# JiGuang283/Ray_Tracing-Rendering

Hardware: AMD Instinct MI355X
Metric: Msamples/sec, Cornell Box 800x800 spp=400 MIS (higher is better)
Workload: dtype f64

## Files before the change

### ray_tracing-rendering_amd/csrc/rt_device.h

```cpp
#pragma once

#include <hip/hip_runtime.h>
#include <stdint.h>

#include "rtr_hip.h"
#include "rtr_seed.h"

#ifndef RTR_BLOCK
#define RTR_BLOCK 256
#endif

#define RT_DEV __device__ __forceinline__
#define RT_HD __host__ __device__ __forceinline__

typedef double Real;

#define RT_STATS_WORDS 80
#define RT_PROF_BASE 8
#define RT_PROF_REGIONS 36
enum { RG_OTHER = 0, RG_SETUP = 1, RG_RECTS = 2, RG_SPHERES = 3, RG_GENERIC = 4, RG_TREE = 5, RG_LEAVES = 6, RG_FINISH = 7,
       RG_SH_SETUP = 8, RG_SH_RECTS = 9, RG_SH_SPHERES = 10, RG_SH_GENERIC = 11, RG_SH_TREE = 12, RG_SH_LEAVES = 13,
       RG_MEDIA = 14, RG_MATPREP = 15, RG_SHADE_A = 16, RG_SHADE_B = 17, RG_MISS = 18, RG_REGEN = 19, RG_SHADE_RR = 20,
       RG_PARK = 21, RG_BARRIER = 22, RG_EXCHANGE = 23, RG_PAIR_SETUP = 24, RG_PAIR_RUNS = 25, RG_PAIR_SPHERES = 26,
       RG_POLL = 27, RG_BEGIN = 28, RG_SETTLE = 29, RG_COUNT = 30, RG_REJECT = 31,
       RG_EMIT_MIS = 32,
       RG_CAMDIV = 33,
       RG_LANE_DIV = 34,
       RG_LANE_SQRT = 35,
       RG_N = 36 };
#ifdef RTR_REGION_PROFILE
__shared__ unsigned long long rt_prof_lds[4 * 2 * RT_PROF_REGIONS + 4 * 2];
RT_DEV void rt_region(int id) {
    const unsigned long long m = __ballot(1);
    if ((int)__lane_id() == __builtin_ctzll(m)) {
        const int w = threadIdx.x >> 6;
        unsigned long long* acc = rt_prof_lds + w * 2 * RT_PROF_REGIONS;
        unsigned long long* st = rt_prof_lds + 4 * 2 * RT_PROF_REGIONS + w * 2;
        const unsigned long long now = __builtin_readcyclecounter();
        acc[st[1]] += now - st[0];
        acc[RT_PROF_REGIONS + id] += 1;
        st[0] = now, st[1] = (unsigned long long)id;
    }
}
RT_DEV int rt_region_current() { return (int)rt_prof_lds[4 * 2 * RT_PROF_REGIONS + (threadIdx.x >> 6) * 2 + 1]; }
#define RT_REGION(id) rt_region(id)
#define RT_REGION_CURRENT() rt_region_current()
#else
#define RT_REGION(id) do { } while (0)
#define RT_REGION_CURRENT() 0
#endif

#define RT_INF (__builtin_huge_val())
// ... 1404 lines not shown
                 ".Lpx%=:\n\t"
                 "s_mov_b64 exec, %[save]"
                 : [u] "=&v"(u), [save] "=&s"(save), [tmaxA] "+v"(tmaxA), [hitA] "+v"(hitA), [tmaxB] "+v"(tmaxB), [hitB] "+v"(hitB)
                 : [tA] "v"(tA), [uA] "v"(uA), [wA] "v"(wA), [tB] "v"(tB), [oaB] "v"(oaB), [daB] "v"(daB), [obB] "v"(obB),
                   [dbB] "v"(dbB), [a0] "s"(a0), [a1] "s"(a1), [b0] "s"(b0), [b1] "s"(b1), [ref] "s"(ref), [tmin] "s"(tmin)
                 : "vcc");
}
struct PairRay {
    V3 o, d;
    RayDiv q;
};
template <int TYPE>
RT_DEV void pair_rects(const RT_CONST_AS double* p, int cnt, int ref, const PairRay& A, Real& tmaxA, int& hitA, const PairRay& B,
                       Real& tmaxB, int& hitB) {
    int k = 0;
    for (; k + 1 < cnt; k += 2, p += 10) {
        const Real f0 = p[0], f1 = p[1], f2 = p[2], f3 = p[3], f4 = p[4];
        const Real g0 = p[5], g1 = p[6], g2 = p[7], g3 = p[8], g4 = p[9];
        pair_rect<TYPE>(f0, f1, f2, f3, f4, ref + k, A.o, A.d, A.q, tmaxA, hitA, B.o, B.d, B.q, tmaxB, hitB);
        pair_rect<TYPE>(g0, g1, g2, g3, g4, ref + k + 1, A.o, A.d, A.q, tmaxA, hitA, B.o, B.d, B.q, tmaxB, hitB);
    }
    if (k < cnt) pair_rect<TYPE>(p[0], p[1], p[2], p[3], p[4], ref + k, A.o, A.d, A.q, tmaxA, hitA, B.o, B.d, B.q, tmaxB, hitB);
}
RT_DEV void pair_runs(const DScene& sc, const FInst& I, const PairRay& A, Real time, Real& tmaxA, int& hitA, const PairRay& B,
                      Real& tmaxB, int& hitB) {
    const RT_CONST_AS double* p = as_const(sc.fscan) + I.scan_first;
    int ref = I.ref_first;
#pragma nounroll
    for (uint64_t runs = I.runs; runs != 0; runs >>= RT_RUN_BITS) {
        const int type = RTR_NODE_SPHERE + (int)((runs >> RT_RUN_COUNT_BITS) & 7), cnt = (int)(runs & RT_RUN_COUNT_MAX);
        RT_REGION(type >= RTR_NODE_XY_RECT ? RG_PAIR_RUNS : RG_PAIR_SPHERES);
        if (type == RTR_NODE_XY_RECT) {
            pair_rects<RTR_NODE_XY_RECT>(p, cnt, ref, A, tmaxA, hitA, B, tmaxB, hitB);
            p += 5 * cnt;
        } else if (type == RTR_NODE_XZ_RECT) {
            pair_rects<RTR_NODE_XZ_RECT>(p, cnt, ref, A, tmaxA, hitA, B, tmaxB, hitB);
            p += 5 * cnt;
        } else if (type == RTR_NODE_YZ_RECT) {
            pair_rects<RTR_NODE_YZ_RECT>(p, cnt, ref, A, tmaxA, hitA, B, tmaxB, hitB);
            p += 5 * cnt;
        } else if (type == RTR_NODE_SPHERE + RT_RUN_BOX) {
            for (int b = 0, r = ref; b < cnt; ++b, p += 6, r += 6) {
                const Real x0 = p[0], x1 = p[1], y0 = p[2], y1 = p[3], z0 = p[4], z1 = p[5];
                pair_rect<RTR_NODE_XY_RECT>(x0, x1, y0, y1, z1, r, A.o, A.d, A.q, tmaxA, hitA, B.o, B.d, B.q, tmaxB, hitB);
                pair_rect<RTR_NODE_XY_RECT>(x0, x1, y0, y1, z0, r + 1, A.o, A.d, A.q, tmaxA, hitA, B.o, B.d, B.q, tmaxB, hitB);
                pair_rect<RTR_NODE_XZ_RECT>(x0, x1, z0, z1, y1, r + 2, A.o, A.d, A.q, tmaxA, hitA, B.o, B.d, B.q, tmaxB, hitB);
                pair_rect<RTR_NODE_XZ_RECT>(x0, x1, z0, z1, y0, r + 3, A.o, A.d, A.q, tmaxA, hitA, B.o, B.d, B.q, tmaxB, hitB);
                pair_rect<RTR_NODE_YZ_RECT>(y0, y1, z0, z1, x1, r + 4, A.o, A.d, A.q, tmaxA, hitA, B.o, B.d, B.q, tmaxB, hitB);
                pair_rect<RTR_NODE_YZ_RECT>(y0, y1, z0, z1, x0, r + 5, A.o, A.d, A.q, tmaxA, hitA, B.o, B.d, B.q, tmaxB, hitB);
            }
            ref += 5 * cnt;
        } else {
            for (int k = 0; k < cnt; ++k, p += 4) {
                const V3 c = mk(p[0], p[1], p[2]);
                const Real r = p[3];
                Real t;
                if (sphere_hit_t<true>(c, r, A.o, A.d, A.q, 0.001, tmaxA, t)) tmaxA = t, hitA = ref + k;
                if (sphere_hit_t<true>(c, r, B.o, B.d, B.q, 0.001, tmaxB, t)) tmaxB = t, hitB = ref + k;
            }
        }
        ref += cnt;
    }
}
struct PairFrame {
    V3 ao, bo;
    Real adx, adz, bdx, bdz;
};
RT_HD void pair_rot(Real s, Real c, Real x, Real z, Real& rx, Real& rz) {
    rx = c * x - s * z;
    rz = s * x + c * z;
}
RT_HD PairFrame pair_frame(int shape, const double* f0, const double* f1, V3 ao, V3 ad, V3 bo, V3 bd) {
    PairFrame F;
    switch (shape) {
    case RT_SHAPE_T:
// ... 11 lines not shown
        const Real ax = ao.x - f0[0], bx = bo.x - f0[0];
        const Real az = ao.z - f0[2], bz = bo.z - f0[2];
        F.ao.y = ao.y - f0[1], F.bo.y = bo.y - f0[1];
        pair_rot(f1[0], f1[1], ax, az, F.ao.x, F.ao.z), pair_rot(f1[0], f1[1], bx, bz, F.bo.x, F.bo.z);
        pair_rot(f1[0], f1[1], ad.x, ad.z, F.adx, F.adz), pair_rot(f1[0], f1[1], bd.x, bd.z, F.bdx, F.bdz);
        break;
    }
    case RT_SHAPE_RT: {
        Real ax, az, bx, bz;
        pair_rot(f0[0], f0[1], ao.x, ao.z, ax, az), pair_rot(f0[0], f0[1], bo.x, bo.z, bx, bz);
        pair_rot(f0[0], f0[1], ad.x, ad.z, F.adx, F.adz), pair_rot(f0[0], f0[1], bd.x, bd.z, F.bdx, F.bdz);
        F.ao.x = ax - f1[0], F.bo.x = bx - f1[0];
        F.ao.y = ao.y - f1[1], F.bo.y = bo.y - f1[1];
        F.ao.z = az - f1[2], F.bo.z = bz - f1[2];
        break;
    }
    default:
        F.ao = ao, F.bo = bo;
        F.adx = ad.x, F.adz = ad.z, F.bdx = bd.x, F.bdz = bd.z;
        break;
    }
    return F;
}
__device__ __forceinline__ void trace_pair(const DScene& sc, V3 ao, V3 ad, Real atime, Real& a_tmax, int& a_ref, int& a_inst,
                                           V3 bo, V3 bd, Real& b_tmax, int& b_ref, const Stack st) {
    a_ref = -1, a_inst = -1, b_ref = -1;
#ifndef RTR_NO_SHARED_DIV
    const bool ok_a = raydiv_origin_ok(ao), ok_b = raydiv_origin_ok(bo);
#else
    const bool ok_a = false, ok_b = false;
#endif
    const Real way = rcp_refined(ad.y), wby = rcp_refined(bd.y);
    const bool wa_y = rcp_safe(ad.y), wb_y = rcp_safe(bd.y);
    for (int ii = 0; ii < sc.n_finst; ++ii) {
        RT_REGION(RG_PAIR_SETUP);
        const FInst I = ld_const(sc.finst, ii);
        PairRay A, B;
        if (I.shape != RT_SHAPE_OTHER) {
            const PairFrame F = pair_frame(I.shape, I.xf_f[0], I.xf_f[1], ao, ad, bo, bd);
            A.o = F.ao, B.o = F.bo;
            A.d = mk(F.adx, ad.y, F.adz), B.d = mk(F.bdx, bd.y, F.bdz);
        } else {
            A.o = ao, A.d = ad, B.o = bo, B.d = bd;
            wrapper_enter(I.xf_type[0], I.xf_f[0], A.o, A.d);
            wrapper_enter(I.xf_type[0], I.xf_f[0], B.o, B.d);
            if (I.n_xf > 1) {
                wrapper_enter(I.xf_type[1], I.xf_f[1], A.o, A.d);
                wrapper_enter(I.xf_type[1], I.xf_f[1], B.o, B.d);
// ... 13 lines not shown
        if (I.flags & RT_INST_SPHERES) {
            A.q.a = len2(A.d), B.q.a = len2(B.d);
            A.q.ra = rcp_refined(A.q.a), B.q.ra = rcp_refined(B.q.a);
            sa = sa & rcp_safe(A.q.a), sb = sb & rcp_safe(B.q.a);
        }
        if (ok_a && ok_b && __all(sa & sb)) {
            A.q.fast = B.q.fast = true;
            pair_runs(sc, I, A, atime, a_tmax, a_ref, B, b_tmax, b_ref);
        } else {
            A.q.fast = ok_a && __all(sa), B.q.fast = ok_b && __all(sb);
            int order = -1;
            if (A.q.fast)
                scan_instance<false, false, false, true>(sc, I, A.o, A.d, A.q, atime, 0.001, a_tmax, a_ref, order, st, 0);
            else
                scan_instance<false, false, false, false>(sc, I, A.o, A.d, A.q, atime, 0.001, a_tmax, a_ref, order, st, 0);
            if (B.q.fast)
                scan_instance<true, false, true, true>(sc, I, B.o, B.d, B.q, 0.0, 0.001, b_tmax, b_ref, order, st, 0);
            else
                scan_instance<true, false, true, false>(sc, I, B.o, B.d, B.q, 0.0, 0.001, b_tmax, b_ref, order, st, 0);
        }
        RT_REGION(RG_PAIR_SETUP);
        if (a_ref >= I.ref_first) a_inst = ii;
    }
}

template <bool UV>
__device__ __forceinline__ void fast_finish_long(const DScene& sc, V3 o, V3 d, Real time, Real t, int ref, int inst, Hit& rec) {
    const FInst I = ld_const(sc.finst, inst);
    const FRef R = ld_const(sc.fref, ref);
    V3 lo = o, ld = d;
    for (int k = 0; k < I.n_xf; ++k) {
        const FXf x = ld_const(sc.fxf, I.xf_first + k);
        wrapper_enter(x.type, x.f, lo, ld);
    }
    const rtr_node n = ld_const(sc.fprim, ref);
    const int type = n.type;
    if (type >= RTR_NODE_XY_RECT) {
        Real oa, da, ob, db;
        if (type == RTR_NODE_XY_RECT) {
            oa = lo.x, da = ld.x, ob = lo.y, db = ld.y;
        } else if (type == RTR_NODE_XZ_RECT) {
            oa = lo.x, da = ld.x, ob = lo.z, db = ld.z;
        } else {
            oa = lo.y, da = ld.y, ob = lo.z, db = ld.z;
        }
        rect_fill(n, type, lo, ld, t, oa + t * da, ob + t * db, UV, rec);
// ... 1166 lines not shown
```

### ray_tracing-rendering_amd/csrc/rt_kernels.h

```cpp
#pragma once

#include "rt_render.h"

#ifndef RTR_MEGA_WAVES
#define RTR_MEGA_WAVES 4
#endif
#ifndef RTR_PROGRAM_WAVES
#define RTR_PROGRAM_WAVES 3
#endif

constexpr int mega_waves(int integ, int trav, int ms) {
    if (ms == RT_MS_LEAN) return RTR_MEGA_WAVES;
    if (rt_is_program(trav)) return RTR_PROGRAM_WAVES;
    if (trav == RT_TRAV_MEDIA || trav == RT_TRAV_EXACT) return 2;
    if (ms == RT_MS_QUADLIT) return 3;
    if (integ == RTR_INTEGRATOR_RR || integ == RTR_INTEGRATOR_PATH) return 3;
    return 2;
}

#define RT_PARK_WORDS 19
struct Park {
    double* base;
    RT_DEV V3 get3(int k) const { return mk(base[k * RTR_BLOCK], base[(k + 1) * RTR_BLOCK], base[(k + 2) * RTR_BLOCK]); }
    RT_DEV void set3(int k, V3 v) const {
        base[k * RTR_BLOCK] = v.x, base[(k + 1) * RTR_BLOCK] = v.y, base[(k + 2) * RTR_BLOCK] = v.z;
    }
    RT_DEV double get(int k) const { return base[k * RTR_BLOCK]; }
    RT_DEV void set(int k, double v) const { base[k * RTR_BLOCK] = v; }
    RT_DEV void get2(int k, uint32_t& lo, uint32_t& hi) const {
        const unsigned long long w = (unsigned long long)__double_as_longlong(base[k * RTR_BLOCK]);
        lo = (uint32_t)w, hi = (uint32_t)(w >> 32);
    }
    RT_DEV void set2(int k, uint32_t lo, uint32_t hi) const {
        base[k * RTR_BLOCK] = __longlong_as_double((long long)((unsigned long long)lo | ((unsigned long long)hi << 32)));
    }
};
enum { PK_THR = 0, PK_L = 3, PK_ACC = 6, PK_PDF = 9, PK_NCAST = 10, PK_PIXEL = 11,
       PK_CONTRIB = 12, PK_SWI = 15, PK_STMAX = 18 };
struct ParkedReq {
    bool valid;
    Park pk;
// ... 300 lines not shown
            RTR_CLK(other);
            RT_REGION(RG_OTHER);
            const bool cast_a = !done;
            Real a_tmax = RT_INF, b_tmax = 0.0;
            int a_ref, a_inst, b_ref;
            V3 swi = mk(1.0, 1.0, 1.0);
            RT_REGION(RG_COUNT);
            {
                uint32_t n_closest, n_shadow;
                pk.get2(PK_NCAST, n_closest, n_shadow);
                pk.set2(PK_NCAST, n_closest + (cast_a ? 1u : 0u), n_shadow + (pending ? 1u : 0u));
            }
            RT_REGION(RG_OTHER);
            if (!cast_a) {
                ps.ro = mk(0.0, 0.0, 0.0), ps.rd = mk(1.0, 1.0, 1.0), ps.tm = 0.0;
                a_tmax = 0.0;
            }
            if (pending) {
                swi = pk.get3(PK_SWI);
                b_tmax = pk.get(PK_STMAX);
            } else {
                so = mk(0.0, 0.0, 0.0);
            }
            trace_pair(sc, ps.ro, ps.rd, ps.tm, a_tmax, a_ref, a_inst, so, swi, b_tmax, b_ref, st);
            RTR_CLK(closest);
            RT_REGION(RG_POLL);
            const uint32_t cancel_word = cancel_poll_issue(P, it++);
            RT_REGION(RG_SETTLE);
            const bool lit = pending && b_ref < 0;
            if (lit || settle) {
                V3 L = pk.get3(PK_L);
                if (lit) L = add(L, pk.get3(PK_CONTRIB));
                if (settle) {
                    pk.set3(PK_ACC, add(pk.get3(PK_ACC), L));
                    if (ACC == 2) {
                        const double y = luminance(L);
                        q += y * y;
                    }
                    L = mk(0.0, 0.0, 0.0);
                    settle = false;
                }
                pk.set3(PK_L, L);
            }
            pending = false;
            RTR_CLK(shadow);
            if (cast_a) {
                bool ended;
// ... 252 lines not shown
        bool now = false;
        if (need && k < RT_QUEUE_JOBS) {
            const int i = tile_x * 16 + (k & 15), j = tile_y * 16 + qb.quarter * 4 + (k >> 4);
            if (i >= P.x0 && i < P.x1 && j >= P.y0 && j < P.y1 && qb.s0 < qb.s1) {
                uint32_t lo, hi;
                queue_pack(i, j, qb.s1, lo, hi);
                pk.set2(PK_PIXEL, lo, hi);
                *my_cell = cell;
                s = qb.s0;
                got = now = true, need = false;
            } else {
                atomicAdd(&P.done[cell], 1);
            }
        }
        qw.samples += (unsigned long long)__builtin_popcountll(__ballot(now)) * (unsigned long long)(qb.s1 - qb.s0);
        const int taken = qw.next + (int)__builtin_popcountll(m);
        qw.next = taken < RT_QUEUE_JOBS ? taken : RT_QUEUE_JOBS;
        m = __ballot(need);
    }
    slot.set(qw);
    return got;
}

template <int INTEG, int TRAV, int MS>
__global__ void __launch_bounds__(RTR_BLOCK, mega_waves(INTEG, TRAV, MS))
    k_mega_queue(const DScene* __restrict__ scp, const RenderK P, const int stack_words, uint32_t* __restrict__ ,
                 const int ) {
    static_assert(mega_pairable(INTEG, TRAV), "no pair-cast variant of this kernel");
    extern __shared__ int lds_stack[];
    const DScene& sc = *scp;
    const Stack st{lds_stack + threadIdx.x};
    const Park pk{reinterpret_cast<double*>(lds_stack + stack_words * RTR_BLOCK) + threadIdx.x};
    int* const my_cell = lds_stack + threadIdx.x;
    const QueueSlot slot;
#ifdef RTR_REGION_PROFILE
    if (threadIdx.x < 4 * 2 * RT_PROF_REGIONS + 8) rt_prof_lds[threadIdx.x] = 0;
    if (threadIdx.x + 256 < 4 * 2 * RT_PROF_REGIONS + 8) rt_prof_lds[threadIdx.x + 256] = 0;
    __syncthreads();
    if ((threadIdx.x & 63) == 0) rt_prof_lds[4 * 2 * RT_PROF_REGIONS + (threadIdx.x >> 6) * 2] = __builtin_readcyclecounter();
#endif
    PathCounters cnt;
    cnt.closest = 0, cnt.shadow = 0;
    PathState ps;
    uint32_t rng = 1;
    int s = 0;
    slot.set(QueueWave{0, RT_QUEUE_JOBS, 0ull});
// ... 23 lines not shown
    bool pending = false;
    bool settle = false;
    V3 so = mk(0.0, 0.0, 0.0);
    PhaseClocks clk;
    while (!done || settle) {
        RTR_CLK(other);
        RT_REGION(RG_OTHER);
        const bool cast_a = !done;
        Real a_tmax = RT_INF;
        int a_ref, a_inst, b_ref;
        RT_REGION(RG_COUNT);
        {
            uint32_t n_closest, n_shadow;
            pk.get2(PK_NCAST, n_closest, n_shadow);
            pk.set2(PK_NCAST, n_closest + (cast_a ? 1u : 0u), n_shadow + (pending ? 1u : 0u));
        }
        RT_REGION(RG_OTHER);
        if (!cast_a) {
            ps.ro = mk(0.0, 0.0, 0.0), ps.rd = mk(1.0, 1.0, 1.0), ps.tm = 0.0;
            a_tmax = 0.0;
        }
        const V3 swi = pk.get3(PK_SWI);
        Real b_tmax = pk.get(PK_STMAX);
        trace_pair(sc, ps.ro, ps.rd, ps.tm, a_tmax, a_ref, a_inst, so, swi, b_tmax, b_ref, st);
        RTR_CLK(closest);
        RT_REGION(RG_POLL);
        const uint32_t cancel_word = cancel_poll_issue(P, it++);
        RT_REGION(RG_SETTLE);
        const bool lit = pending && b_ref < 0;
        if (lit || settle) {
            V3 L = pk.get3(PK_L);
            if (lit) L = add(L, pk.get3(PK_CONTRIB));
            if (settle) {
                pk.set3(PK_ACC, add(pk.get3(PK_ACC), L));
                L = mk(0.0, 0.0, 0.0);
                settle = false;
            }
            pk.set3(PK_L, L);
        }
        pending = false;
        {
            Real dead = 0.0;
            asm volatile("" : "+v"(dead));
            pk.set(PK_STMAX, dead);
        }
        RTR_CLK(shadow);
        bool begin = false;
// ... 542 lines not shown
```

### ray_tracing-rendering_amd/csrc/rt_test_kernels.h

```cpp
#pragma once

#include "rt_kernels.h"
#include "rtr_hip_test.h"
#include "rtr_testrec.h"

template <int TRAV>
__global__ void __launch_bounds__(RTR_BLOCK) k_test_hits(const DScene sc, rtr_hit_record* recs, long long n) {
    extern __shared__ int lds_stack[];
    const Stack st{lds_stack + threadIdx.x};
    const long long k = (long long)blockIdx.x * RTR_BLOCK + threadIdx.x;
    if (k >= n) return;
    rtr_hit_record r = recs[k];
    uint32_t rng = r.rng_in;
    Hit rec;
    rec.u = rec.v = __builtin_nan("");
    rec.mat = -1;
    rec.t = 0, rec.p = mk(0, 0, 0), rec.n = mk(0, 0, 0), rec.front = false;
    Real tmax = r.t_max;
    bool h;
    if (TRAV == RT_TRAV_FAST || TRAV == RT_TRAV_TOP) {
        int ref, inst;
        h = trace_fast<false, true, false, TRAV == RT_TRAV_TOP>(sc, sub_scene0(sc), ld3(r.o), ld3(r.d), r.time, r.t_min, tmax, ref, inst, st, 0);
        if (h) fast_finish<true>(sc, ld3(r.o), ld3(r.d), r.time, tmax, ref, inst, rec);
    } else if (rt_is_program(TRAV)) {
// ... 18 lines not shown
    extern __shared__ int lds_stack[];
    const Stack st{lds_stack + threadIdx.x};
    const long long k = (long long)blockIdx.x * RTR_BLOCK + threadIdx.x;
    if (k >= n) return;
    rtr_hit_record r = recs[k];
    uint32_t rng = r.rng_in;
    Hit rec;
    rec.u = rec.v = __builtin_nan("");
    rec.mat = -1;
    rec.t = 0, rec.p = mk(0, 0, 0), rec.n = mk(0, 0, 0), rec.front = false;
    const bool h = cast_closest<TRAV>(sc, ld3(r.o), ld3(r.d), r.time, rec, rng, st, r.t_min, r.t_max);
    r.rng_out = rng;
    r.hit = h;
    r.front_face = h ? (int)rec.front : 0;
    r.material = h ? rec.mat : -1;
    r.pad = 0;
    r.t = h ? rec.t : 0;
    r.p[0] = h ? rec.p.x : 0, r.p[1] = h ? rec.p.y : 0, r.p[2] = h ? rec.p.z : 0;
    r.n[0] = h ? rec.n.x : 0, r.n[1] = h ? rec.n.y : 0, r.n[2] = h ? rec.n.z : 0;
    r.u = h ? rec.u : 0, r.v = h ? rec.v : 0;
    recs[k] = r;
}

__global__ void __launch_bounds__(RTR_BLOCK) k_test_pair(const DScene sc, rtr_pair_record* recs, long long n) {
    extern __shared__ int lds_stack[];
    const Stack st{lds_stack + threadIdx.x};
    const long long k = (long long)blockIdx.x * RTR_BLOCK + threadIdx.x;
    if (k >= n) return;
    rtr_pair_record r = recs[k];
    Real a_t = r.a_tmax, b_t = r.b_tmax;
    int a_ref, a_inst, b_ref;
    trace_pair(sc, ld3(r.ao), ld3(r.ad), 0.0, a_t, a_ref, a_inst, ld3(r.bo), ld3(r.bd), b_t, b_ref, st);
    Real s_t = r.a_tmax, sb_t = r.b_tmax;
    int s_ref, s_inst, sb_ref, sb_inst;
    trace_fast<false, false, false, false, false>(sc, sub_scene0(sc), ld3(r.ao), ld3(r.ad), 0.0, 0.001, s_t, s_ref, s_inst, st, 0);
    trace_fast<true, false, true, false, false>(sc, sub_scene0(sc), ld3(r.bo), ld3(r.bd), 0.0, 0.001, sb_t, sb_ref, sb_inst, st, 0);
    r.a_t = a_t, r.s_a_t = s_t;
    r.a_ref = a_ref, r.a_inst = a_inst, r.b_hit = b_ref >= 0;
    r.s_a_ref = s_ref, r.s_a_inst = s_inst, r.s_b_hit = sb_ref >= 0;
    recs[k] = r;
}

RT_DEV bool same_bits(Real a, Real b) { return (a != a && b != b) || __double_as_longlong(a) == __double_as_longlong(b); }

template <int MS>
__global__ void __launch_bounds__(RTR_BLOCK) k_test_materials(const DScene sc, rtr_mat_record* recs, long long n) {
    const long long k = (long long)blockIdx.x * RTR_BLOCK + threadIdx.x;
    if (k >= n) return;
    rtr_mat_record r = recs[k];
    Hit rec;
    rec.p = ld3(r.p), rec.n = ld3(r.n);
    rec.u = r.u, rec.v = r.v, rec.t = 1.0;
    rec.front = r.front_face != 0;
    rec.mat = r.material;
    const V3 wo = ld3(r.wo), wi = ld3(r.wi_in);
    uint32_t rng = r.rng_in;
    BSDFSample bs;
    bs.wi = mk(0, 0, 0), bs.f = mk(0, 0, 0), bs.pdf = 0, bs.is_specular = false, bs.is_transmission = false;
    const MatCtx mc = mat_prepare<MS>(sc, rec);
    const UDiv pi = scene_pi(sc);
    const bool ok = mat_sample<MS>(mc, rec, wo, bs, rng, pi);
// ... 298 lines not shown
```

### ray_tracing-rendering_amd/csrc/rtr_capi.hip

```cpp
#include "rt_context.h"
#include "rt_render_kernels.h"
#include "rt_validate.h"

#include <cstdio>
#include <cstring>

using namespace rtr;

static thread_local std::string g_create_error;

namespace rtr {

int fail(rtr_context* c, int code, const std::string& msg) {
    if (c)
        c->err = msg;
    else
        g_create_error = msg;
    return code;
}

int ensure(rtr_context* c, DevBuf& b, size_t bytes) {
    if (bytes == 0) bytes = 16;
    if (b.cap >= bytes) return RTR_OK;
    if (b.p) {
// ... 73 lines not shown
            c->in_flight = false;
            HIPCHK(c, hipStreamSynchronize(c->stream));
        }
        return RTR_OK;
    }
    HIPCHK(c, hipEventSynchronize(c->ev1));
    float ms = 0;
    HIPCHK(c, hipEventElapsedTime(&ms, c->ev0, c->ev1));
    unsigned long long h[RT_STATS_WORDS] = {0};
    HIPCHK(c, hipMemcpy(h, c->b_stats.p, sizeof h, hipMemcpyDeviceToHost));
    if (getenv("RTR_REGION_PROFILE")) {
        static const char* names[RG_N] = {"other / loop", "closest: instance setup", "closest: rect runs", "closest: sphere runs",
                                          "closest: generic scan", "closest: tree inner nodes", "closest: tree leaves",
                                          "closest: hit record (fast_finish)", "shadow: instance setup", "shadow: rect runs",
                                          "shadow: sphere runs", "shadow: generic scan", "shadow: tree inner nodes",
                                          "shadow: tree leaves", "media steps", "mat_prepare", "shade_a (emission, light sample)",
                                          "shade_b (BSDF sample, roulette)", "miss", "end of sample + regeneration",
                                          "shade_rr / shade_path", "park path state", "sorted shading: barrier waits",
                                          "sorted shading: tickets + exchange / queue: job switch", "pair cast: instance setup",
                                          "pair cast: rect runs", "pair cast: sphere runs", "sample end: cancel poll",
                                          "sample end: begin_sample (camera ray)", "sample end: settle into the pixel sum",
                                          "cast counters", "random_in_unit_sphere rejection loop",
                                          "shade_a: emitter MIS weight (compute_light_pdf)", "camera_sample: image-size divisions",
                                          "shading: lane-varying 1 / x and n / d", "shading: lane-varying sqrt"};
        double total = 0;
        for (int k = 0; k < RG_N; ++k) total += (double)h[RT_PROF_BASE + k];
        std::fprintf(stderr, "[region profile] %.4g wave cycles in all, %llu samples\n", total, h[0]);
        for (int k = 0; k < RG_N; ++k)
            if (h[RT_PROF_BASE + RT_PROF_REGIONS + k])
                std::fprintf(stderr, "[region profile] %-48s %6.2f %%  %12llu visits  %8.1f cycles/visit\n", names[k],
                             100.0 * (double)h[RT_PROF_BASE + k] / total, h[RT_PROF_BASE + RT_PROF_REGIONS + k],
                             (double)h[RT_PROF_BASE + k] / (double)h[RT_PROF_BASE + RT_PROF_REGIONS + k]);
    }
#ifdef RTR_PHASE_CLOCKS
    std::fprintf(stderr, "[phase clocks] closest %.3e  shade %.3e  shadow %.3e  other %.3e (wave cycles)\n", (double)h[3],
                 (double)h[4], (double)h[5], (double)h[6]);
#endif
    c->stats.samples = h[0];
    c->stats.closest_segments = h[1];
    c->stats.shadow_segments = h[2];
    c->stats.device_ms = ms;
    if (h[7]) c->stats.cancelled = 1;
    c->stats_pending = false;
    c->in_flight = false;
    return RTR_OK;
}

// ... 616 lines not shown
```

### ray_tracing-rendering_amd/native.py

```python
import ctypes as C
import os
import weakref

import numpy as np

from . import _abi as A
from .scene import Scene

_HERE = os.path.dirname(os.path.abspath(__file__))
_LIB = None

_STATUS = {A.RTR_ERR_INVALID: "RTR_ERR_INVALID", A.RTR_ERR_UNSUPPORTED: "RTR_ERR_UNSUPPORTED",
           A.RTR_ERR_DEVICE: "RTR_ERR_DEVICE", A.RTR_ERR_NO_SCENE: "RTR_ERR_NO_SCENE",
           A.RTR_ERR_CANCELLED: "RTR_ERR_CANCELLED", A.RTR_ERR_NOMEM: "RTR_ERR_NOMEM"}

EXPORTS = ("rtr_abi_version", "rtr_device_count", "rtr_create", "rtr_destroy", "rtr_set_stream",
           "rtr_upload_scene", "rtr_render_device", "rtr_render_host", "rtr_render_tiles_host", "rtr_plan_chunks", "rtr_li_samples", "rtr_li_rays",
           "rtr_synchronize", "rtr_cancel", "rtr_get_stats", "rtr_last_error", "rtr_sample_seed", "rtr_validate_scene",
           "rtr_accum_create", "rtr_accum_render", "rtr_accum_resolve", "rtr_accum_tiles", "rtr_accum_destroy",
           "rtr_accum_create_ex", "rtr_accum_render_tiles", "rtr_accum_moments", "rtr_accum_errors", "rtr_accum_refine",
           "rtr_denoise_defaults", "rtr_accum_features", "rtr_accum_denoise", "rtr_denoise_host",
           "rtr_query_closest", "rtr_query_occluded", "rtr_query_closest_device", "rtr_query_occluded_device",
           "rtr_set_camera", "rtr_get_camera", "rtr_accum_reset", "rtr_temporal_defaults", "rtr_history_create",
           "rtr_history_clear", "rtr_history_destroy", "rtr_history_planes", "rtr_accum_denoise_temporal",
           "rtr_display_defaults", "rtr_display_srgb_thresholds", "rtr_display_histogram", "rtr_display_host",
           "rtr_display_device", "rtr_accum_resolve_device", "rtr_accum_features_device", "rtr_accum_denoise_device",
           "rtr_accum_denoise_temporal_device", "rtr_gather_defaults", "rtr_gather_occlusion", "rtr_gather_radiance",
           "rtr_gather_occlusion_device", "rtr_gather_radiance_device", "rtr_gather_ray",
           "rtr_probe_visibility", "rtr_probe_radiance", "rtr_probe_visibility_device", "rtr_probe_radiance_device",
           "rtr_probe_ray", "rtr_sh_basis", "rtr_sh_irradiance", "rtr_probe_lookup", "rtr_probe_lookup_device",
           "rtr_probe_lookup_one", "rtr_capture_defaults", "rtr_capture_cube", "rtr_capture_cube_device", "rtr_capture_ray",
           "rtr_cube_lookup", "rtr_cube_lookup_device", "rtr_cube_lookup_one", "rtr_latlong_direction",
           "rtr_cube_to_latlong", "rtr_write_rgbe", "rtr_cube_filter_defaults", "rtr_cube_filter", "rtr_cube_filter_device",
           "rtr_cube_filter_one", "rtr_cube_chain_plan", "rtr_cube_chain_lookup", "rtr_cube_chain_lookup_device",
           "rtr_cube_chain_lookup_one", "rtr_probe_depth_defaults", "rtr_probe_depth", "rtr_probe_depth_device",
           "rtr_probe_depth_ray", "rtr_octa_encode", "rtr_octa_decode", "rtr_probe_lookup_visible",
           "rtr_probe_lookup_visible_device", "rtr_probe_lookup_visible_one")
TEST_EXPORTS = ("rtr_test_hits", "rtr_test_materials", "rtr_test_lights", "rtr_test_li", "rtr_test_reference_order",
                "rtr_test_stream8", "rtr_test_sincos_exhaustive", "rtr_test_shared_division", "rtr_test_issue_rates", "rtr_test_last_kernel",
                "rtr_test_last_gather", "rtr_test_last_probe", "rtr_test_last_capture", "rtr_test_last_probe_depth",
                "rtr_test_temporal_planes", "rtr_test_scene_plan", "rtr_test_flat_hits", "rtr_test_pair_frames",
                "rtr_test_pair_frame_host", "rtr_test_pair_cast", "rtr_test_queue_blocks_host", "rtr_test_queue_pack_host",
                "rtr_test_scatter", "rtr_test_materials_ms", "rtr_test_scatter_ms", "rtr_test_lights_ms", "rtr_test_pow5",
                "rtr_test_pow5_host", "rtr_test_udiv", "rtr_test_scene_consts", "rtr_test_accum_load",
                "rtr_test_accum_plan", "rtr_test_accum_commit", "rtr_test_rcp_lane", "rtr_test_sqrt_lane",
                "rtr_test_lane_specials", "rtr_test_lane_host", "rtr_test_draw_forms", "rtr_test_draw_callers",
                "rtr_test_draw_host", "rtr_test_draw_host_range")
_TEST_LIB = None


class SceneInfoC(C.Structure):
    _fields_ = [("stack_words", C.c_int32), ("has_media", C.c_int32), ("needs_uv", C.c_int32),
                ("graph_depth", C.c_int32), ("fast_ok", C.c_int32), ("fast_instances", C.c_int32),
                ("fast_refs", C.c_int32), ("fast_stack_words", C.c_int32), ("compiled_subtrees", C.c_int32),
                ("program_steps", C.c_int32), ("inverted_boxes", C.c_int32), ("top_trees", C.c_int32)]


class KernelRecordC(C.Structure):
    _fields_ = [(name, C.c_int32) for name in ("pipeline", "integrator", "trav", "ms", "sorted", "shade_phases", "lean",
                                               "quadlit", "sort", "media", "machine", "accum", "pair", "queue")]


class GatherRecordC(C.Structure):
    _fields_ = [(name, C.c_int32) for name in ("integ", "trav", "broadcast", "lg")]

# ... 6 lines not shown
    _fields_ = [(name, C.c_int32) for name in ("integ", "trav", "lg")]


class ProbeDepthRecordC(C.Structure):
    _fields_ = [(name, C.c_int32) for name in ("trav", "lg")]


class ScenePlanC(C.Structure):
    _fields_ = [(name, C.c_int32) for name in (
        "fast_ok", "has_media", "flat_scene", "flat_guarded", "lean_materials", "quad_lights_only", "uv_order_dependent",
        "machine_ok", "guarded_program", "top_tree", "needs_uv", "n_material_types", "shared_div", "pair_cast", "n_steps",
        "n_visits", "n_refs", "fast_stack_words", "walk_stack_words", "n_tie_refs", "n_guard_refs", "pick_trav", "mega_trav",
        "mega_ms", "mega_sorted", "mega_pair", "n_finish")]


FINISH_DTYPE = np.dtype([("kind", "<i4"), ("material", "<i4"), ("levels", "<i4"), ("flip", "<i4"), ("op", "<f8", (2, 3)),
                         ("g", "<f8", (4,))])


PAIR_FRAME_DTYPE = np.dtype([("ao", "<f8", (3,)), ("ad", "<f8", (3,)), ("bo", "<f8", (3,)), ("bd", "<f8", (3,)),
                             ("fo", "<f8", (3,)), ("fd", "<f8", (3,)), ("same_frame", "<i4"), ("pad", "<i4")])
PAIR_DTYPE = np.dtype([("ao", "<f8", (3,)), ("ad", "<f8", (3,)), ("a_tmax", "<f8"), ("bo", "<f8", (3,)), ("bd", "<f8", (3,)),
                       ("b_tmax", "<f8"), ("a_t", "<f8"), ("s_a_t", "<f8"), ("a_ref", "<i4"), ("a_inst", "<i4"),
                       ("b_hit", "<i4"), ("s_a_ref", "<i4"), ("s_a_inst", "<i4"), ("s_b_hit", "<i4")])
QUEUE_BLOCK_DTYPE = np.dtype([(name, "<i4") for name in ("slot", "quarter", "chunk", "s0", "s1", "ref_s0", "ref_s1", "pad")])
MS_LEAN, MS_FULL, MS_QUADLIT = 0, 1, 2
FRAME_SHAPES = ("none", "T", "R", "TR", "RT", "other")


class RtrError(RuntimeError):
    def __init__(self, code, message):
        super().__init__("%s (%d): %s" % (_STATUS.get(code, "rtr_status"), code, message))
        self.code = code
        self.message = message


def library_path():
    return os.environ.get("RTR_HIP_LIBRARY") or os.path.join(_HERE, "librtr_hip.so")


def lib():
    global _LIB
    if _LIB is not None:
        return _LIB
    path = library_path()
    if not os.path.exists(path):
        raise RtrError(A.RTR_ERR_DEVICE, "HIP library %s is missing: run __graft_entry__.build(); there is no "
# ... 136 lines not shown
    for name in ("rtr_test_materials_ms", "rtr_test_scatter_ms", "rtr_test_lights_ms"):
        getattr(T, name).argtypes = [vp, vp, C.c_int64, C.c_int32]
    T.rtr_test_pow5.argtypes = [vp, vp, vp, C.c_int64]
    T.rtr_test_pow5_host.argtypes = [vp, vp, C.c_int64]
    T.rtr_test_li.argtypes = [vp, C.POINTER(A.RenderParamsC), vp, C.c_int64]
    T.rtr_test_reference_order.argtypes = [vp, C.c_int]
    T.rtr_test_stream8.argtypes = [vp, C.c_int64, C.c_int]
    T.rtr_test_sincos_exhaustive.argtypes = [vp, C.POINTER(C.c_uint64), C.POINTER(C.c_uint64)]
    T.rtr_test_issue_rates.argtypes = [vp, C.POINTER(C.c_double), C.c_int]
    T.rtr_test_shared_division.argtypes = [vp, C.POINTER(C.c_uint64), C.POINTER(C.c_uint64)]
    T.rtr_test_last_kernel.argtypes = [vp, C.POINTER(KernelRecordC), C.c_size_t]
    T.rtr_test_last_gather.argtypes = [vp, C.POINTER(GatherRecordC), C.c_size_t]
    T.rtr_test_last_probe.argtypes = [vp, C.POINTER(ProbeRecordC), C.c_size_t]
    T.rtr_test_last_capture.argtypes = [vp, C.POINTER(CaptureRecordC), C.c_size_t]
    T.rtr_test_last_probe_depth.argtypes = [vp, C.POINTER(ProbeDepthRecordC), C.c_size_t]
    T.rtr_test_temporal_planes.argtypes = [vp] + [C.c_int32] * 6 + [C.POINTER(A.CameraC), C.POINTER(A.CameraC), C.c_int,
                                                                    C.POINTER(A.TemporalParamsC)] + [vp] * 8
    T.rtr_test_scene_plan.argtypes = [C.POINTER(A.SceneDescC), C.c_int32, C.c_int32, C.POINTER(ScenePlanC), vp, C.c_int64,
                                      vp, C.c_int64]
    T.rtr_test_flat_hits.argtypes = [vp, vp, C.c_int64, C.c_int, C.POINTER(C.c_int32)]
    T.rtr_test_pair_frames.argtypes = [C.POINTER(A.SceneDescC), vp, C.c_int64, C.POINTER(C.c_int32)]
    T.rtr_test_pair_frame_host.argtypes = [C.c_int32, vp, vp, C.c_int64]
    T.rtr_test_pair_cast.argtypes = [vp, vp, C.c_int64]
    T.rtr_test_queue_blocks_host.argtypes = [C.c_int32] * 6 + [vp, C.c_int64]
    T.rtr_test_queue_pack_host.argtypes = [C.c_int32] * 3 + [C.POINTER(C.c_uint32), C.POINTER(C.c_uint32), vp]
    T.rtr_test_udiv.argtypes = [vp, vp, C.c_int64, vp, C.c_int32, C.POINTER(C.c_uint64), C.POINTER(C.c_uint64)]
    T.rtr_test_scene_consts.argtypes = [vp, vp, vp, C.c_int64, C.POINTER(C.c_int32)]
    for name in ("rtr_test_rcp_lane", "rtr_test_sqrt_lane"):
        getattr(T, name).argtypes = [vp] + [C.POINTER(C.c_uint64)] * 3 + [vp]
    T.rtr_test_lane_specials.argtypes = [vp, C.c_int64]
    T.rtr_test_lane_host.argtypes = [C.c_int32, C.c_int32, vp, vp, vp, C.c_int64]
    T.rtr_test_draw_forms.argtypes = [vp] + [C.POINTER(C.c_uint64)] * 3
    T.rtr_test_draw_callers.argtypes = [vp, C.c_uint64, C.c_int64] + [C.POINTER(C.c_uint64)] * 3
    T.rtr_test_draw_host.argtypes = [vp, vp, C.c_int64]
    T.rtr_test_draw_host_range.argtypes = [C.c_uint64, C.c_uint64, C.c_uint64, C.c_int32, C.POINTER(C.c_uint64), C.POINTER(C.c_uint64)]
    T.rtr_test_accum_load.argtypes = [vp, vp, vp, vp, vp, C.c_int64]
    T.rtr_test_accum_plan.argtypes = [vp, C.c_int64] + [C.c_int32] * 4 + [C.c_double, vp, vp, vp, vp, C.POINTER(C.c_int32)]
    T.rtr_test_accum_commit.argtypes = [vp, C.c_int64, vp, C.c_int32] + [vp] * 7
    _TEST_LIB = T
    return T


def validate_scene(scene):
    L = lib()
    d = scene.desc()
    info = SceneInfoC()
# ... 1026 lines not shown
        sum_ = np.array(sum, dtype=np.float64, order="C")
        cnt = np.array(count, dtype=np.int32, order="C")
        if any(a.shape != (n,) for a in ints) or cnt.shape != (n,) or partial.shape != (n, 3, 256) or sum_.shape != (n, 3, 256):
            raise ValueError("n tiles: int arrays (n,), partial and sum (n, 3, 256) expected")
        if (q is None) != (q_part is None):
            raise ValueError("q and q_part go together")
        qq = qp = None
        if q is not None:
            qp = np.ascontiguousarray(q_part, dtype=np.float64)
            qq = np.array(q, dtype=np.float64, order="C")
            if qp.shape != (n, 256) or qq.shape != (n, 256):
                raise ValueError("q_part and q of shape (n, 256) expected")
        self._chk(test_lib().rtr_test_accum_commit(
            self._h, n, ints[0].ctypes.data, int(n_active), ints[1].ctypes.data, ints[2].ctypes.data, partial.ctypes.data,
            None if qp is None else qp.ctypes.data, sum_.ctypes.data, None if qq is None else qq.ctypes.data, cnt.ctypes.data))
        return sum_, qq, cnt

    def flat_hits(self, recs, with_uv=True):
        out = np.ascontiguousarray(recs.copy())
        used = C.c_int32(0)
        self._chk(test_lib().rtr_test_flat_hits(self._h, out.ctypes.data, len(out), 1 if with_uv else 0, C.byref(used)))
        return out, bool(used.value)

    def pair_cast(self, ao, ad, bo, bd, a_tmax=np.inf, b_tmax=np.inf):
        recs = np.zeros(len(ao), dtype=PAIR_DTYPE)
        recs["ao"], recs["ad"], recs["bo"], recs["bd"] = ao, ad, bo, bd
        recs["a_tmax"], recs["b_tmax"] = a_tmax, b_tmax
        self._chk(test_lib().rtr_test_pair_cast(self._h, recs.ctypes.data, len(recs)))
        return recs

    def test_records(self, kind, recs, params=None, ms=None):
        out = np.ascontiguousarray(recs.copy())
        if kind == "pow5":
            x = np.ascontiguousarray(recs, dtype=np.float64)
            out = np.zeros_like(x)
            self._chk(test_lib().rtr_test_pow5(self._h, x.ctypes.data, out.ctypes.data, x.size))
            return out
        if ms is not None:
            fn = getattr(test_lib(), "rtr_test_%s_ms" % kind)
            self._chk(fn(self._h, out.ctypes.data, len(out), int(ms)))
            return out
        fn = getattr(test_lib(), "rtr_test_" + kind)
        if kind == "li":
            self._chk(fn(self._h, C.byref(params), out.ctypes.data, len(out)))
        else:
            self._chk(fn(self._h, out.ctypes.data, len(out)))
        return out


class Accumulator:

# ... 200 lines not shown
```

Baseline: 6073.

## Add lean pair-cast path that bails to single casts when fast-division checks fail

Result: faster. 6215, median of 6 (+2.3%).

```diff
diff --git a/ray_tracing-rendering_amd/csrc/rt_device.h b/ray_tracing-rendering_amd/csrc/rt_device.h
--- a/ray_tracing-rendering_amd/csrc/rt_device.h
+++ b/ray_tracing-rendering_amd/csrc/rt_device.h
@@ -15,9 +15,9 @@
 
 typedef double Real;
 
-#define RT_STATS_WORDS 80
+#define RT_STATS_WORDS 82
 #define RT_PROF_BASE 8
-#define RT_PROF_REGIONS 36
+#define RT_PROF_REGIONS 37
 enum { RG_OTHER = 0, RG_SETUP = 1, RG_RECTS = 2, RG_SPHERES = 3, RG_GENERIC = 4, RG_TREE = 5, RG_LEAVES = 6, RG_FINISH = 7,
        RG_SH_SETUP = 8, RG_SH_RECTS = 9, RG_SH_SPHERES = 10, RG_SH_GENERIC = 11, RG_SH_TREE = 12, RG_SH_LEAVES = 13,
        RG_MEDIA = 14, RG_MATPREP = 15, RG_SHADE_A = 16, RG_SHADE_B = 17, RG_MISS = 18, RG_REGEN = 19, RG_SHADE_RR = 20,
@@ -27,7 +27,8 @@
        RG_CAMDIV = 33,
        RG_LANE_DIV = 34,
        RG_LANE_SQRT = 35,
-       RG_N = 36 };
+       RG_PAIR_RECAST = 36,
+       RG_N = 37 };
 #ifdef RTR_REGION_PROFILE
 __shared__ unsigned long long rt_prof_lds[4 * 2 * RT_PROF_REGIONS + 4 * 2];
 RT_DEV void rt_region(int id) {
@@ -1478,6 +1479,7 @@
     }
     if (k < cnt) pair_rect<TYPE>(p[0], p[1], p[2], p[3], p[4], ref + k, A.o, A.d, A.q, tmaxA, hitA, B.o, B.d, B.q, tmaxB, hitB);
 }
+template <bool SPHERES = true>
 RT_DEV void pair_runs(const DScene& sc, const FInst& I, const PairRay& A, Real time, Real& tmaxA, int& hitA, const PairRay& B,
                       Real& tmaxB, int& hitB) {
     const RT_CONST_AS double* p = as_const(sc.fscan) + I.scan_first;
@@ -1506,7 +1508,7 @@
                 pair_rect<RTR_NODE_YZ_RECT>(y0, y1, z0, z1, x0, r + 5, A.o, A.d, A.q, tmaxA, hitA, B.o, B.d, B.q, tmaxB, hitB);
             }
             ref += 5 * cnt;
-        } else {
+        } else if (SPHERES) {
             for (int k = 0; k < cnt; ++k, p += 4) {
                 const V3 c = mk(p[0], p[1], p[2]);
                 const Real r = p[3];
@@ -1564,8 +1566,8 @@
     }
     return F;
 }
-__device__ __forceinline__ void trace_pair(const DScene& sc, V3 ao, V3 ad, Real atime, Real& a_tmax, int& a_ref, int& a_inst,
-                                           V3 bo, V3 bd, Real& b_tmax, int& b_ref, const Stack st) {
+__device__ __forceinline__ bool trace_pair_frames(const DScene& sc, V3 ao, V3 ad, Real atime, Real& a_tmax, int& a_ref, int& a_inst,
+                                                  V3 bo, V3 bd, Real& b_tmax, int& b_ref, const Stack st) {
     a_ref = -1, a_inst = -1, b_ref = -1;
 #ifndef RTR_NO_SHARED_DIV
     const bool ok_a = raydiv_origin_ok(ao), ok_b = raydiv_origin_ok(bo);
@@ -1625,6 +1627,100 @@
         RT_REGION(RG_PAIR_SETUP);
         if (a_ref >= I.ref_first) a_inst = ii;
     }
+    return true;
+}
+typedef unsigned long long PairMask;
+RT_DEV PairMask pair_within(Real x, Real lo, Real hi) {
+    PairMask a, b;
+    asm volatile("v_cmp_ge_f64_e64 %0, |%2|, %3\n\tv_cmp_le_f64_e64 %1, |%2|, %4" : "=&s"(a), "=&s"(b) : "v"(x), "s"(lo), "s"(hi));
+    return a & b;
+}
+RT_DEV PairMask pair_safe(Real d) { return pair_within(d, 0x1p-100, 0x1p100); }
+RT_DEV PairMask pair_below(Real x, Real hi) {
+    PairMask a;
+    asm volatile("v_cmp_le_f64_e64 %0, |%1|, %2" : "=s"(a) : "v"(x), "s"(hi));
+    return a;
+}
+RT_DEV PairMask pair_origin_in(V3 o) { return pair_below(o.x, 0x1p80) & pair_below(o.y, 0x1p80) & pair_below(o.z, 0x1p80); }
+RT_DEV bool pair_vote(PairMask m) { return m == __builtin_amdgcn_read_exec(); }
+RT_DEV bool pair_scan(const DScene& sc, const FInst& I, V3 ao, Real adx, Real ady, Real adz, Real way, V3 bo, Real bdx, Real bdy,
+                      Real bdz, Real wby, PairMask sy, Real atime, Real& a_tmax, int& a_ref, Real& b_tmax, int& b_ref) {
+    PairRay A, B;
+    A.o = ao, B.o = bo;
+    A.d = mk(adx, ady, adz), B.d = mk(bdx, bdy, bdz);
+    A.q.guard = B.q.guard = false;
+    A.q.fast = B.q.fast = true;
+    A.q.rx = rcp_refined(adx), A.q.rz = rcp_refined(adz);
+    B.q.rx = rcp_refined(bdx), B.q.rz = rcp_refined(bdz);
+    A.q.ry = way, B.q.ry = wby;
+    A.q.a = A.q.ra = B.q.a = B.q.ra = 0;
+    const PairMask s = pair_safe(adx) & pair_safe(adz) & pair_safe(bdx) & pair_safe(bdz) & sy;
+    if (I.flags & RT_INST_SPHERES) {
+        Real ayy, byy;
+        asm volatile("v_mul_f64 %0, %2, %2\n\tv_mul_f64 %1, %3, %3" : "=&v"(ayy), "=&v"(byy) : "v"(ady), "v"(bdy));
+        A.q.a = adx * adx + ayy + adz * adz, B.q.a = bdx * bdx + byy + bdz * bdz;
+        A.q.ra = rcp_refined(A.q.a), B.q.ra = rcp_refined(B.q.a);
+        if (!pair_vote(s & pair_safe(A.q.a) & pair_safe(B.q.a))) return false;
+        pair_runs<true>(sc, I, A, atime, a_tmax, a_ref, B, b_tmax, b_ref);
+    } else {
+        if (!pair_vote(s)) return false;
+        pair_runs<false>(sc, I, A, atime, a_tmax, a_ref, B, b_tmax, b_ref);
+    }
+    return true;
+}
+__device__ __forceinline__ bool trace_pair_recast(const DScene& sc, V3 ao, V3 ad, Real atime, Real& a_tmax, int& a_ref, int& a_inst,
+                                                  V3 bo, V3 bd, Real& b_tmax, int& b_ref) {
+    a_ref = -1, a_inst = -1, b_ref = -1;
+#ifdef RTR_NO_SHARED_DIV
+    return false;
+#endif
+    if (!pair_vote(pair_origin_in(ao) & pair_origin_in(bo))) return false;
+    const Real way = rcp_refined(ad.y), wby = rcp_refined(bd.y);
+    const PairMask sy = pair_safe(ad.y) & pair_safe(bd.y);
+    for (int ii = 0; ii < sc.n_finst; ++ii) {
+        RT_REGION(RG_PAIR_SETUP);
+        const FInst I = ld_const(sc.finst, ii);
+        PairFrame F;
+        if (I.shape != RT_SHAPE_OTHER) {
+            F = pair_frame(I.shape, I.xf_f[0], I.xf_f[1], ao, ad, bo, bd);
+        } else {
+            V3 fad = ad, fbd = bd;
+            F.ao = ao, F.bo = bo;
+            wrapper_enter(I.xf_type[0], I.xf_f[0], F.ao, fad);
+            wrapper_enter(I.xf_type[0], I.xf_f[0], F.bo, fbd);
+            if (I.n_xf > 1) {
+                wrapper_enter(I.xf_type[1], I.xf_f[1], F.ao, fad);
+                wrapper_enter(I.xf_type[1], I.xf_f[1], F.bo, fbd);
+            }
+            for (int k = RT_INST_XF_INLINE; k < I.n_xf; ++k) {
+                const FXf x = ld_const(sc.fxf, I.xf_first + k);
+                wrapper_enter(x.type, x.f, F.ao, fad);
+                wrapper_enter(x.type, x.f, F.bo, fbd);
+            }
+            F.adx = fad.x, F.adz = fad.z, F.bdx = fbd.x, F.bdz = fbd.z;
+        }
+        if (!pair_scan(sc, I, F.ao, F.adx, ad.y, F.adz, way, F.bo, F.bdx, bd.y, F.bdz, wby, sy, atime, a_tmax, a_ref, b_tmax, b_ref))
+            return false;
+        RT_REGION(RG_PAIR_SETUP);
+        if (a_ref >= I.ref_first) a_inst = ii;
+    }
+    return true;
+}
+template <bool RECAST = true>
+__device__ __forceinline__ bool trace_pair(const DScene& sc, V3 ao, V3 ad, Real atime, Real& a_tmax, int& a_ref, int& a_inst,
+                                           V3 bo, V3 bd, Real& b_tmax, int& b_ref, const Stack st) {
+#ifndef RTR_PAIR_FRAME_FALLBACK
+    if (RECAST) return trace_pair_recast(sc, ao, ad, atime, a_tmax, a_ref, a_inst, bo, bd, b_tmax, b_ref);
+#endif
+    return trace_pair_frames(sc, ao, ad, atime, a_tmax, a_ref, a_inst, bo, bd, b_tmax, b_ref, st);
+}
+RT_DEV void pair_recast(const DScene& sc, V3 ao, V3 ad, Real atime, Real& a_tmax, int& a_ref, int& a_inst, V3 bo, V3 bd,
+                        Real& b_tmax, int& b_ref, const Stack st) {
+    RT_REGION(RG_PAIR_RECAST);
+    int b_inst;
+    const FSub sub = sub_scene0(sc);
+    trace_fast<false, false, false, false, false>(sc, sub, ao, ad, atime, 0.001, a_tmax, a_ref, a_inst, st, 0);
+    trace_fast<true, false, true, false, false>(sc, sub, bo, bd, 0.0, 0.001, b_tmax, b_ref, b_inst, st, 0);
 }
 
 template <bool UV>
diff --git a/ray_tracing-rendering_amd/csrc/rt_kernels.h b/ray_tracing-rendering_amd/csrc/rt_kernels.h
--- a/ray_tracing-rendering_amd/csrc/rt_kernels.h
+++ b/ray_tracing-rendering_amd/csrc/rt_kernels.h
@@ -17,6 +17,8 @@
     if (integ == RTR_INTEGRATOR_RR || integ == RTR_INTEGRATOR_PATH) return 3;
     return 2;
 }
+
+constexpr bool pair_recasts(int ms) { return ms == RT_MS_LEAN; }
 
 #define RT_PARK_WORDS 19
 struct Park {
@@ -363,7 +365,11 @@
             } else {
                 so = mk(0.0, 0.0, 0.0);
             }
-            trace_pair(sc, ps.ro, ps.rd, ps.tm, a_tmax, a_ref, a_inst, so, swi, b_tmax, b_ref, st);
+            if (!trace_pair<pair_recasts(MS)>(sc, ps.ro, ps.rd, ps.tm, a_tmax, a_ref, a_inst, so, swi, b_tmax, b_ref, st)) {
+                a_tmax = cast_a ? RT_INF : 0.0;
+                b_tmax = pending ? pk.get(PK_STMAX) : 0.0;
+                pair_recast(sc, ps.ro, ps.rd, ps.tm, a_tmax, a_ref, a_inst, so, swi, b_tmax, b_ref, st);
+            }
             RTR_CLK(closest);
             RT_REGION(RG_POLL);
             const uint32_t cancel_word = cancel_poll_issue(P, it++);
@@ -662,6 +668,11 @@
     return got;
 }
 
+RT_DEV void pair_retire(const Park& pk, V3& so) {
+    pk.set3(PK_SWI, mk(1.0, 1.0, 1.0));
+    so = mk(0.0, 0.0, 0.0);
+}
+
 template <int INTEG, int TRAV, int MS>
 __global__ void __launch_bounds__(RTR_BLOCK, mega_waves(INTEG, TRAV, MS))
     k_mega_queue(const DScene* __restrict__ scp, const RenderK P, const int stack_words, uint32_t* __restrict__ ,
@@ -731,7 +742,12 @@
         }
         const V3 swi = pk.get3(PK_SWI);
         Real b_tmax = pk.get(PK_STMAX);
-        trace_pair(sc, ps.ro, ps.rd, ps.tm, a_tmax, a_ref, a_inst, so, swi, b_tmax, b_ref, st);
+        if (!trace_pair<pair_recasts(MS)>(sc, ps.ro, ps.rd, ps.tm, a_tmax, a_ref, a_inst, so, swi, b_tmax, b_ref, st)) {
+            a_tmax = cast_a ? RT_INF : 0.0;
+            b_tmax = pk.get(PK_STMAX);
+            pair_recast(sc, ps.ro, ps.rd, ps.tm, a_tmax, a_ref, a_inst, so, swi, b_tmax, b_ref, st);
+            pair_retire(pk, so);
+        }
         RTR_CLK(closest);
         RT_REGION(RG_POLL);
         const uint32_t cancel_word = cancel_poll_issue(P, it++);
diff --git a/ray_tracing-rendering_amd/csrc/rt_test_kernels.h b/ray_tracing-rendering_amd/csrc/rt_test_kernels.h
--- a/ray_tracing-rendering_amd/csrc/rt_test_kernels.h
+++ b/ray_tracing-rendering_amd/csrc/rt_test_kernels.h
@@ -64,6 +64,7 @@
     recs[k] = r;
 }
 
+template <bool RECAST>
 __global__ void __launch_bounds__(RTR_BLOCK) k_test_pair(const DScene sc, rtr_pair_record* recs, long long n) {
     extern __shared__ int lds_stack[];
     const Stack st{lds_stack + threadIdx.x};
@@ -72,13 +73,58 @@
     rtr_pair_record r = recs[k];
     Real a_t = r.a_tmax, b_t = r.b_tmax;
     int a_ref, a_inst, b_ref;
-    trace_pair(sc, ld3(r.ao), ld3(r.ad), 0.0, a_t, a_ref, a_inst, ld3(r.bo), ld3(r.bd), b_t, b_ref, st);
+    r.recasts = 0, r.pad = 0;
+    if (!trace_pair<RECAST>(sc, ld3(r.ao), ld3(r.ad), 0.0, a_t, a_ref, a_inst, ld3(r.bo), ld3(r.bd), b_t, b_ref, st)) {
+        a_t = r.a_tmax, b_t = r.b_tmax;
+        pair_recast(sc, ld3(r.ao), ld3(r.ad), 0.0, a_t, a_ref, a_inst, ld3(r.bo), ld3(r.bd), b_t, b_ref, st);
+        r.recasts = 1;
+    }
     Real s_t = r.a_tmax, sb_t = r.b_tmax;
     int s_ref, s_inst, sb_ref, sb_inst;
     trace_fast<false, false, false, false, false>(sc, sub_scene0(sc), ld3(r.ao), ld3(r.ad), 0.0, 0.001, s_t, s_ref, s_inst, st, 0);
     trace_fast<true, false, true, false, false>(sc, sub_scene0(sc), ld3(r.bo), ld3(r.bd), 0.0, 0.001, sb_t, sb_ref, sb_inst, st, 0);
     r.a_t = a_t, r.s_a_t = s_t;
     r.a_ref = a_ref, r.a_inst = a_inst, r.b_hit = b_ref >= 0;
+    r.s_a_ref = s_ref, r.s_a_inst = s_inst, r.s_b_hit = sb_ref >= 0;
+    recs[k] = r;
+}
+
+__global__ void __launch_bounds__(RTR_BLOCK) k_test_pair_resident(const DScene sc, rtr_pair_record* recs, long long n,
+                                                                  const int stack_words, const int casts) {
+    extern __shared__ int lds_stack[];
+    const Stack st{lds_stack + threadIdx.x};
+    const Park pk{reinterpret_cast<double*>(lds_stack + stack_words * RTR_BLOCK) + threadIdx.x};
+    const long long k = (long long)blockIdx.x * RTR_BLOCK + threadIdx.x;
+    if (k >= n) return;
+    rtr_pair_record r = recs[k];
+    const V3 ao = ld3(r.ao), ad = ld3(r.ad);
+    V3 so = ld3(r.bo);
+    pk.set3(PK_SWI, ld3(r.bd));
+    pk.set(PK_STMAX, r.b_tmax);
+    r.recasts = 0, r.pad = 0;
+    for (int c = 0; c < casts; ++c) {
+        Real a_t = r.a_tmax;
+        int a_ref, a_inst, b_ref;
+        const V3 swi = pk.get3(PK_SWI);
+        Real b_t = pk.get(PK_STMAX);
+        if (!trace_pair(sc, ao, ad, 0.0, a_t, a_ref, a_inst, so, swi, b_t, b_ref, st)) {
+            a_t = r.a_tmax;
+            b_t = pk.get(PK_STMAX);
+            pair_recast(sc, ao, ad, 0.0, a_t, a_ref, a_inst, so, swi, b_t, b_ref, st);
+            pair_retire(pk, so);
+            ++r.recasts;
+        }
+        pk.set(PK_STMAX, 0.0);
+        if (c == 0) {
+            r.a_t = a_t;
+            r.a_ref = a_ref, r.a_inst = a_inst, r.b_hit = b_ref >= 0;
+        }
+    }
+    Real s_t = r.a_tmax, sb_t = r.b_tmax;
+    int s_ref, s_inst, sb_ref, sb_inst;
+    trace_fast<false, false, false, false, false>(sc, sub_scene0(sc), ao, ad, 0.0, 0.001, s_t, s_ref, s_inst, st, 0);
+    trace_fast<true, false, true, false, false>(sc, sub_scene0(sc), ld3(r.bo), ld3(r.bd), 0.0, 0.001, sb_t, sb_ref, sb_inst, st, 0);
+    r.s_a_t = s_t;
     r.s_a_ref = s_ref, r.s_a_inst = s_inst, r.s_b_hit = sb_ref >= 0;
     recs[k] = r;
 }
diff --git a/ray_tracing-rendering_amd/csrc/rtr_capi.hip b/ray_tracing-rendering_amd/csrc/rtr_capi.hip
--- a/ray_tracing-rendering_amd/csrc/rtr_capi.hip
+++ b/ray_tracing-rendering_amd/csrc/rtr_capi.hip
@@ -119,7 +119,8 @@
                                           "sample end: begin_sample (camera ray)", "sample end: settle into the pixel sum",
                                           "cast counters", "random_in_unit_sphere rejection loop",
                                           "shade_a: emitter MIS weight (compute_light_pdf)", "camera_sample: image-size divisions",
-                                          "shading: lane-varying 1 / x and n / d", "shading: lane-varying sqrt"};
+                                          "shading: lane-varying 1 / x and n / d", "shading: lane-varying sqrt",
+                                          "pair cast: recast through the single casts"};
         double total = 0;
         for (int k = 0; k < RG_N; ++k) total += (double)h[RT_PROF_BASE + k];
         std::fprintf(stderr, "[region profile] %.4g wave cycles in all, %llu samples\n", total, h[0]);
diff --git a/ray_tracing-rendering_amd/native.py b/ray_tracing-rendering_amd/native.py
--- a/ray_tracing-rendering_amd/native.py
+++ b/ray_tracing-rendering_amd/native.py
@@ -40,7 +40,7 @@
                 "rtr_test_stream8", "rtr_test_sincos_exhaustive", "rtr_test_shared_division", "rtr_test_issue_rates", "rtr_test_last_kernel",
                 "rtr_test_last_gather", "rtr_test_last_probe", "rtr_test_last_capture", "rtr_test_last_probe_depth",
                 "rtr_test_temporal_planes", "rtr_test_scene_plan", "rtr_test_flat_hits", "rtr_test_pair_frames",
-                "rtr_test_pair_frame_host", "rtr_test_pair_cast", "rtr_test_queue_blocks_host", "rtr_test_queue_pack_host",
+                "rtr_test_pair_frame_host", "rtr_test_pair_cast", "rtr_test_pair_cast_text", "rtr_test_pair_resident", "rtr_test_queue_blocks_host", "rtr_test_queue_pack_host",
                 "rtr_test_scatter", "rtr_test_materials_ms", "rtr_test_scatter_ms", "rtr_test_lights_ms", "rtr_test_pow5",
                 "rtr_test_pow5_host", "rtr_test_udiv", "rtr_test_scene_consts", "rtr_test_accum_load",
                 "rtr_test_accum_plan", "rtr_test_accum_commit", "rtr_test_rcp_lane", "rtr_test_sqrt_lane",
@@ -93,7 +93,9 @@
                              ("fo", "<f8", (3,)), ("fd", "<f8", (3,)), ("same_frame", "<i4"), ("pad", "<i4")])
 PAIR_DTYPE = np.dtype([("ao", "<f8", (3,)), ("ad", "<f8", (3,)), ("a_tmax", "<f8"), ("bo", "<f8", (3,)), ("bd", "<f8", (3,)),
                        ("b_tmax", "<f8"), ("a_t", "<f8"), ("s_a_t", "<f8"), ("a_ref", "<i4"), ("a_inst", "<i4"),
-                       ("b_hit", "<i4"), ("s_a_ref", "<i4"), ("s_a_inst", "<i4"), ("s_b_hit", "<i4")])
+                       ("b_hit", "<i4"), ("s_a_ref", "<i4"), ("s_a_inst", "<i4"), ("s_b_hit", "<i4"), ("recasts", "<i4"),
+                       ("pad", "<i4")])
+assert PAIR_DTYPE.itemsize == 160
 QUEUE_BLOCK_DTYPE = np.dtype([(name, "<i4") for name in ("slot", "quarter", "chunk", "s0", "s1", "ref_s0", "ref_s1", "pad")])
 MS_LEAN, MS_FULL, MS_QUADLIT = 0, 1, 2
 FRAME_SHAPES = ("none", "T", "R", "TR", "RT", "other")
@@ -276,6 +278,8 @@
     T.rtr_test_pair_frames.argtypes = [C.POINTER(A.SceneDescC), vp, C.c_int64, C.POINTER(C.c_int32)]
     T.rtr_test_pair_frame_host.argtypes = [C.c_int32, vp, vp, C.c_int64]
     T.rtr_test_pair_cast.argtypes = [vp, vp, C.c_int64]
+    T.rtr_test_pair_cast_text.argtypes = [vp, vp, C.c_int64, C.c_int32]
+    T.rtr_test_pair_resident.argtypes = [vp, vp, C.c_int64, C.c_int32]
     T.rtr_test_queue_blocks_host.argtypes = [C.c_int32] * 6 + [vp, C.c_int64]
     T.rtr_test_queue_pack_host.argtypes = [C.c_int32] * 3 + [C.POINTER(C.c_uint32), C.POINTER(C.c_uint32), vp]
     T.rtr_test_udiv.argtypes = [vp, vp, C.c_int64, vp, C.c_int32, C.POINTER(C.c_uint64), C.POINTER(C.c_uint64)]
@@ -1348,11 +1352,18 @@
         self._chk(test_lib().rtr_test_flat_hits(self._h, out.ctypes.data, len(out), 1 if with_uv else 0, C.byref(used)))
         return out, bool(used.value)
 
-    def pair_cast(self, ao, ad, bo, bd, a_tmax=np.inf, b_tmax=np.inf):
+    def pair_cast(self, ao, ad, bo, bd, a_tmax=np.inf, b_tmax=np.inf, recast=True):
         recs = np.zeros(len(ao), dtype=PAIR_DTYPE)
         recs["ao"], recs["ad"], recs["bo"], recs["bd"] = ao, ad, bo, bd
         recs["a_tmax"], recs["b_tmax"] = a_tmax, b_tmax
-        self._chk(test_lib().rtr_test_pair_cast(self._h, recs.ctypes.data, len(recs)))
+        self._chk(test_lib().rtr_test_pair_cast_text(self._h, recs.ctypes.data, len(recs), 1 if recast else 0))
+        return recs
+
+    def pair_resident(self, ao, ad, bo, bd, a_tmax=np.inf, b_tmax=np.inf, casts=1):
+        recs = np.zeros(len(ao), dtype=PAIR_DTYPE)
+        recs["ao"], recs["ad"], recs["bo"], recs["bd"] = ao, ad, bo, bd
+        recs["a_tmax"], recs["b_tmax"] = a_tmax, b_tmax
+        self._chk(test_lib().rtr_test_pair_resident(self._h, recs.ctypes.data, len(recs), casts))
         return recs
 
     def test_records(self, kind, recs, params=None, ms=None):
```
